# prip-lab/MSU-LatentAFIS

Measured on AMD Instinct MI355X. Metric: latent queries/sec vs 100k rolled gallery, higher is better.
Workload: dtype f32

## Files before the change

include/afis_matcher_taps.h:

```cpp
#ifndef AFIS_MATCHER_TAPS_H
#define AFIS_MATCHER_TAPS_H

#include "afis_matcher.h"

#ifdef __cplusplus
extern "C" {
#endif

int afis_debug_lut(afis_ctx* ctx, const afis_template_view* query, float* out, int32_t* n_rows);
int afis_debug_texture_rowmax(afis_ctx* ctx, const afis_template_view* query, int64_t g,
                              float* val, int32_t* arg, int32_t* n_rows);

int afis_debug_stage_list(afis_ctx* ctx, const afis_template_view* query, int64_t g, int which, int stage,
                          float* sim, int32_t* li, int32_t* ri, int32_t* n);

int afis_debug_atan2_grid(afis_ctx* ctx, int R, float* out);

int afis_debug_graph_arith(afis_ctx* ctx, unsigned long long* out8);
int afis_debug_refine_stats(afis_ctx* ctx, unsigned long long* out8, int reset);

int afis_debug_compact_stats(afis_ctx* ctx, long long* out2);

int afis_debug_rank_subjects(afis_ctx* ctx, afis_subjects* subjects, const float* scores , int n_q, int k,
                             int64_t* subject_id, float* subject_score, int64_t* best_idx);

int afis_debug_rank_hits(afis_ctx* ctx, afis_subjects* subjects, const float* scores , int n_q, float min_score, int cap,
                         int64_t* n_hits , int64_t* out_a , float* out_score , int64_t* out_b );

int afis_debug_rank_latent_hits(afis_ctx* ctx, const float* scores , int n_q, float min_score, int cap, int64_t latent_base,
                                int64_t* n_hits , int64_t* latent_idx , float* score );
int afis_debug_rank_rows(afis_ctx* ctx, afis_subset* subset, const float* scores , int n_q, int k,
                         int64_t* topk_idx , float* topk_score );
int afis_debug_transpose_stats(afis_ctx* ctx, long long* out2);

int afis_debug_phase_cycles(afis_ctx* ctx, unsigned long long* out32, int reset);

#ifdef __cplusplus
}
#endif
#endif
```

msu-latentafis_amd/csrc/afis_taps.cpp:

```cpp
#include "afis_ctx.h"
#include "../../include/afis_matcher_taps.h"

using namespace afis;

static int ensure_codes_cf(afis_ctx* ctx, Shard& sh, int variant)
{
    if ((variant != 6 && variant != 7) || sh.codes_cf_built) return AFIS_OK;
    const int64_t G = sh.gal.G;
    std::vector<int32_t> to((size_t)G + 1), cfb((size_t)G + 1);
    HIPCHK(ctx, hipMemcpyAsync(to.data(), sh.gal.tex_off, to.size() * 4, hipMemcpyDeviceToHost, ctx->stream));
    HIPCHK(ctx, hipStreamSynchronize(ctx->stream));
    int64_t nblk = 0;
    for (int64_t t = 0; t < G; ++t) { cfb[(size_t)t] = (int32_t)nblk; const int64_t n = to[(size_t)t + 1] - to[(size_t)t]; nblk += n > 0 ? (n + 63) / 64 + 1 : 0; }
    cfb[(size_t)G] = (int32_t)nblk;
    if (nblk > 0x7fffffff / 64) return fail(ctx, AFIS_EINVAL, "adc_variant 6 / 7: shard too large for the direct kernel's code stream; split the gallery into more shards");
    HIPCHK(ctx, upload(sh.g_tex_cf_blk, cfb, ctx->stream));
    HIPCHK(ctx, sh.g_tex_codes_cf.ensure(std::max<size_t>((size_t)nblk * 64 * 16, 16)));
    sh.gal.tex_cf_blk = sh.g_tex_cf_blk.as<int32_t>();
    sh.gal.tex_codes_cf = sh.g_tex_codes_cf.as<uint4>();
    HIPCHK(ctx, launch_codes_cf(sh.gal, sh.g_tex_codes_cf.p, ctx->stream));
    HIPCHK(ctx, hipStreamSynchronize(ctx->stream));
    sh.codes_cf_built = true;
    return AFIS_OK;
}

static int direct_rowmax(afis_ctx* ctx, const QueryDev& d, const GalleryDev& g, int variant, int chunk, hipEvent_t after_lut)
{
    HIPCHK(ctx, ctx->lut.ensure(std::max<size_t>((size_t)d.n_tiles * kTileFloats * 4, 16)));
    HIPCHK(ctx, launch_lut_build(d, ctx->codewords.as<float>(), ctx->lut.as<float>(), variant, ctx->stream));
    if (after_lut) HIPCHK(ctx, hipEventRecord(after_lut, ctx->stream));
    HIPCHK(ctx, launch_adc_rowmax(d, g, ctx->lut.as<float>(), chunk, variant, ctx->rm_val.as<float>(), ctx->rm_arg.as<int32_t>(), ctx->stream));
    return AFIS_OK;
}

static int direct_adc_stage(afis_ctx* ctx, Shard& sh, const QueryDev& d, int chunk, hipEvent_t after_lut)
{
    const int rcf = ensure_codes_cf(ctx, sh, ctx->adc_variant);
    if (rcf != AFIS_OK) return rcf;
    return direct_rowmax(ctx, d, sh.gal, ctx->adc_variant, chunk, after_lut);
}
__attribute__((constructor)) static void set_direct_adc_stage() { g_direct_adc_stage = direct_adc_stage; }

extern "C" {

int afis_debug_phase_cycles(afis_ctx* ctx, unsigned long long* out32, int reset)
{
    if (!ctx || !out32) return AFIS_EINVAL;
    HIPCHK(ctx, hipSetDevice(ctx->device));
    HIPCHK(ctx, hipStreamSynchronize(ctx->stream));
    HIPCHK(ctx, read_phase_cycles(out32, reset != 0));
    unsigned long long gph[16];
    HIPCHK(ctx, read_graph_phase_cycles(gph, reset != 0));
    for (int i = 0; i < 8; ++i) { out32[5 + i] = gph[i]; out32[21 + i] = gph[8 + i]; }
    return AFIS_OK;
}

int afis_debug_refine_stats(afis_ctx* ctx, unsigned long long* out8, int reset)
{
    if (!ctx || !out8) return fail(ctx, AFIS_EINVAL, "afis_debug_refine_stats: bad argument");
    HIPCHK(ctx, hipSetDevice(ctx->device));
    HIPCHK(ctx, hipStreamSynchronize(ctx->stream));
    for (int i = 0; i < 8; ++i) out8[i] = 0;
    if (!ctx->mf_stats.p) return AFIS_OK;
    HIPCHK(ctx, hipMemcpy(out8, ctx->mf_stats.p, 64, hipMemcpyDeviceToHost));
    if (reset) HIPCHK(ctx, hipMemset(ctx->mf_stats.p, 0, 64));
    return AFIS_OK;
}

int afis_debug_compact_stats(afis_ctx* ctx, long long* out2)
{
    if (!ctx || !out2) return fail(ctx, AFIS_EINVAL, "afis_debug_compact_stats: bad argument");
    out2[0] = ctx->compact_us; out2[1] = ctx->compact_bytes;
    return AFIS_OK;
}

int afis_debug_rank_subjects(afis_ctx* ctx, afis_subjects* subjects, const float* scores, int n_q, int k, int64_t* subject_id, float* subject_score, int64_t* best_idx)
// ... 227 lines not shown
```

msu-latentafis_amd/csrc/graph.hip:

```cpp
#include "afis_device.h"
#include <type_traits>
#include "atan2f_libm.h"
#include "graph_arith.h"
#include "stdsort_order.h"

namespace afis {

#define AFIS_PI 3.1415926
typedef unsigned long long u64;

#ifdef AFIS_PHASE_TIMING
__device__ u64 g_graph_phase[16];
#define GPH_INIT() u64 gph_t0 = __builtin_readcyclecounter()
#define GPH(i) do { if (threadIdx.x == 0) { const u64 t1_ = __builtin_readcyclecounter(); sm.ph[(i)] += t1_ - gph_t0; gph_t0 = t1_; } } while (0)
#define GPH_T0() const u64 gph_k0 = __builtin_readcyclecounter()
#define GPH_K(i) do { if (threadIdx.x == 0) sm.ph[(i)] += __builtin_readcyclecounter() - gph_k0; } while (0)
#define GPH_ZERO() do { if (threadIdx.x < 16) sm.ph[threadIdx.x] = 0; WSYNC(); } while (0)
#define GPH_FLUSH() do { WSYNC(); if (threadIdx.x < 16 && sm.ph[threadIdx.x]) atomicAdd(&g_graph_phase[threadIdx.x], sm.ph[threadIdx.x]); } while (0)
#else
#define GPH_INIT() do {} while (0)
#define GPH(i) do {} while (0)
#define GPH_T0() do {} while (0)
#define GPH_K(i) do {} while (0)
#define GPH_ZERO() do {} while (0)
// ... 301 lines not shown
    }
    dist = fabsf(d1 - d2);
    return ok;
}
template <bool LOOKUP>
__device__ __forceinline__ bool pair_compatible(const Pt& a, const Pt& o, const float* __restrict__ table)
{
    float s1, s2; bool ok = true;
    if (LOOKUP) {
        const int dx1 = abs(a.lx - o.lx), dx2 = abs(a.rx - o.rx), dy1 = abs(a.ly - o.ly), dy2 = abs(a.ry - o.ry);
        ok = !((dx1 >= kDistN) | (dx2 >= kDistN) | (dy1 >= kDistN) | (dy2 >= kDistN));
        s1 = (float)(256 * (dx1 * dx1 + dy1 * dy1)); s2 = (float)(256 * (dx2 * dx2 + dy2 * dy2));
    } else {
        const float dx1 = (float)(a.lx - o.lx), dx2 = (float)(a.rx - o.rx), dy1 = (float)(a.ly - o.ly), dy2 = (float)(a.ry - o.ry);
        const float p = dx1 * dx1, q = dy1 * dy1, r = dx2 * dx2, s = dy2 * dy2;
        s1 = p + q; s2 = r + s;
    }
    const float d1 = __builtin_amdgcn_sqrtf(s1), d2 = __builtin_amdgcn_sqrtf(s2);
    const float dist = fabsf(d1 - d2);
    const float slack = fmaxf(d1, d2) * 4.76837158e-7f;
    if (fabsf(dist - 30.0f) > slack) return ok && dist < 30.0f;
    float exact;
    pair_dist<LOOKUP>(a, o, table, exact);
    return ok && exact < 30.0f;
}
template <bool RANGE_TEST>
__device__ __forceinline__ bool tex_pair_dist(int2 a, int2 o, float& dist)
{
    float n1, n2;
    pair_n(a, o, n1, n2);
    dist = 16.0f * fabsf(sqrt_rn_int(n1) - sqrt_rn_int(n2));
    return RANGE_TEST ? tex_in_range(a, o) : true;
}
template <bool RANGE_TEST>
__device__ __forceinline__ bool tex_pair_compatible(int2 a, int2 o)
{
    float n1, n2;
    pair_n(a, o, n1, n2);
    const bool ok = RANGE_TEST ? tex_in_range(a, o) : true;
    return pair_compatible_n<true>(n1, n2) && ok;
}

__device__ __forceinline__ float minu_pair_dist(int2 a, int2 o)
{
    float n1, n2;
    pair_n(a, o, n1, n2);
    return fabsf(sqrt_rn_int(n1) - sqrt_rn_int(n2));
}
__device__ __forceinline__ bool minu_pair_compatible(int2 a, int2 o)
{
    float n1, n2;
    pair_n(a, o, n1, n2);
    return pair_compatible_n<false>(n1, n2);
}

__device__ __forceinline__ float h_of_x(float x)
{
    const float q0 = x * 0.04f;
    const float r = fmaf(-q0, 25.0f, x);
    const float h = fmaf(r, 0.04f, q0);
    return __builtin_amdgcn_fmed3f(h, 0.0f, 1.0f);
}
__device__ __forceinline__ float h_value(float dist)
{
    const float x = 30.0f - dist;
    const float q0 = x * 0.04f;
    const float r = fmaf(-q0, 25.0f, x);
    const float h = fmaf(r, 0.04f, q0);
    return __builtin_amdgcn_fmed3f(h, 0.0f, 1.0f);
}

template <class SM, bool LOOKUP, int ITERS, int MODE, int REF_TIE>
__device__ int dist_filter(SM& sm, int num, const float* __restrict__ table, const float* __restrict__ ext, SlabBuf slab)
{
    constexpr bool fast = MODE > 0;
    constexpr bool range_test = MODE == 1;
    auto compat_fast = [](int2 a, int2 o) -> bool { if (LOOKUP) return tex_pair_compatible<range_test>(a, o); return minu_pair_compatible(a, o); };
    auto dist_fast = [](int2 a, int2 o) -> float { float d; if (LOOKUP) { tex_pair_dist<range_test>(a, o, d); return d; } return minu_pair_dist(a, o); };
    constexpr int U = SM::U, W = SM::W, NMAX = SM::NMAX;
    [[maybe_unused]] constexpr int PH = LOOKUP ? 8 : 0;
    GPH_INIT();
    const int lane = threadIdx.x;
    for (int i = lane; i < num * W; i += 64) sm.hb[i / W][i % W] = 0u;
    int2 me[U];
#pragma unroll
    for (int u = 0; u < U; ++u) {
        const int t = lane + 64 * u;
        if (t < SM::N4) { sm.b[t] = t < num ? list_sim(sm, ext, t) : 0.0f; sm.y.cc[t] = 0.0f; }
        me[u] = t < num ? sm.xy[t] : make_int2(0, 0);
    }
    WSYNC();
    const int half = num >> 1;
    const bool even = !(num & 1);
    uint32_t* const hb0 = &sm.hb[0][0];
    auto pair = [&](int2 own, int t, int k, int2 other) {
        if (fast ? compat_fast(own, other) : pair_compatible<LOOKUP>(unpack_xy(own), unpack_xy(other), table)) {
            atomicOr(hb0 + (t * W + (k >> 5)), 1u << (k & 31));
            atomicOr(hb0 + (__umul24(k, W) + (t >> 5)), 1u << (t & 31));
        }
    };
    const int tail0 = num & ~63, R = num - tail0;
    const bool grouped = R > 0 && R <= 32;
    const int n_wide = grouped ? tail0 : num;
    uint32_t kb[U];
    const uint32_t num8 = (uint32_t)num * 8u;
#pragma unroll
    for (int u = 0; u < U; ++u) { const int t = lane + 64 * u; kb[u] = t < num ? (uint32_t)t * 8u : 0u; }
#ifndef AFIS_PAIR_UNROLL
#define AFIS_PAIR_UNROLL 1
#endif
    constexpr int DU = fast ? AFIS_PAIR_UNROLL : 1;
    auto pair_loop = [&](auto ua_tag) {
    constexpr int UA = decltype(ua_tag)::value;
    for (int d = 1; d <= half; d += DU) {
        int2 other[DU][UA];
        int kk[DU][UA];
#pragma unroll
        for (int s2 = 0; s2 < DU; ++s2) {
#pragma unroll
            for (int u = 0; u < UA; ++u) {
                const uint32_t a = kb[u] + 8u;
                kb[u] = min(a, a - num8);
                other[s2][u] = *reinterpret_cast<const int2*>(reinterpret_cast<const char*>(sm.xy) + kb[u]);
                kk[s2][u] = (int)(kb[u] >> 3);
            }
        }
        __builtin_amdgcn_sched_barrier(0);
        if (fast) {
            float n1[DU][UA], n2[DU][UA]; bool hit[DU][UA], near[DU][UA]; bool any_near = false;
#pragma unroll
            for (int s2 = 0; s2 < DU; ++s2) {
#pragma unroll
                for (int u = 0; u < UA; ++u) {
                    pair_n(me[u], other[s2][u], n1[s2][u], n2[s2][u]);
                    hit[s2][u] = pair_compatible_t<LOOKUP>(n1[s2][u], n2[s2][u], near[s2][u]);
                    hit[s2][u] = hit[s2][u] | near[s2][u];
                }
            }
            (void)any_near;
#pragma unroll
            for (int s2 = 0; s2 < DU; ++s2) {
                const bool last = d + s2 == half && even;
#pragma unroll
                for (int u = 0; u < UA; ++u) {
                    const int t = lane + 64 * u, k = kk[s2][u];
                    bool ok = hit[s2][u] && t < n_wide && d + s2 <= half && !(last && t >= half);
                    if (LOOKUP && range_test) ok = ok && tex_in_range(me[u], other[s2][u]);
                    if constexpr (LOOKUP) {
                        const int ts = t < num ? t : 0;
                        atomicOr(hb0 + (ts * W + (k >> 5)), ok ? 1u << (k & 31) : 0u);
                        atomicOr(hb0 + (__umul24(k, W) + (ts >> 5)), ok ? 1u << (ts & 31) : 0u);
                    } else if (ok) {
                        atomicOr(hb0 + (t * W + (k >> 5)), 1u << (k & 31));
                        atomicOr(hb0 + (__umul24(k, W) + (t >> 5)), 1u << (t & 31));
                    }
                }
            }
        } else {
            const bool last = d == half && even;
#pragma unroll
            for (int u = 0; u < UA; ++u) {
                const int t = lane + 64 * u;
                if (t < n_wide && !(last && t >= half)) pair(me[u], t, kk[0][u], other[0][u]);
            }
        }
    }
    };
    const int n_blk = (n_wide + 63) >> 6;
    if (n_blk >= U) pair_loop(std::integral_constant<int, U>{});
    else if (U > 1 && n_blk == U - 1) pair_loop(std::integral_constant<int, (U > 1 ? U - 1 : 1)>{});
    else if (n_blk > 0) pair_loop(std::integral_constant<int, U>{});
    if (grouped) {
        const int sh = R <= 8 ? 3 : R <= 16 ? 4 : 5, RG = 1 << sh, dstep = 64 >> sh;
        const int r = lane & (RG - 1), t = tail0 + r;
        const bool row = r < R;
        const int2 own = row ? sm.xy[t] : make_int2(0, 0);
        int d = 1 + (lane >> sh);
        int k = t + d; k = k >= num ? k - num : k;
        for (int d0 = 1; d0 <= half; d0 += dstep) {
            if (row && d <= half && !(d == half && even && t >= half)) pair(own, t, k, sm.xy[k]);
            d += dstep; k += dstep; k = k >= num ? k - num : k;
        }
    }
    WSYNC();
    GPH(PH + 0);
    int myrow[U], trip[U], rlen[U];
    const int Wn = (num + 31) / 32;
    {
        int cnt[U];
#pragma unroll
        for (int u = 0; u < U; ++u) {
            const int t = lane + 64 * u;
            int c = -1;
            if (t < num) {
                c = 0; for (int w = 0; w < Wn; ++w) c += __popc(sm.hb[t][w]);
                sm.y.os.sel[t] = (short)c;
                c = min(c >> 2, 15);
            }
            cnt[u] = c;
        }
        int base = 0;
        for (int bk = 15; bk >= 0; --bk) {
#pragma unroll
            for (int u = 0; u < U; ++u) {
                const bool in = cnt[u] == bk;
                const u64 m = __ballot(in);
                if (in) sm.y.os.order[base + g_lane_prefix(m)] = (short)(lane + 64 * u);
                base += __popcll(m);
            }
        }
        WSYNC();
#pragma unroll
        for (int u = 0; u < U; ++u) {
            const int p = lane + 64 * u;
            myrow[u] = p < num ? (int)sm.y.os.order[p] : -1;
            rlen[u] = myrow[u] >= 0 ? (int)sm.y.os.sel[myrow[u]] : 0;
// ... 685 lines not shown
```

msu-latentafis_amd/csrc/graph_arith.h:

```cpp
#pragma once
#include "afis_device.h"

namespace afis {

typedef short ga_v2s16 __attribute__((ext_vector_type(2)));
typedef unsigned short ga_v2u16 __attribute__((ext_vector_type(2)));

typedef _Float16 ga_v2h __attribute__((ext_vector_type(2)));

__device__ __forceinline__ int pack_h2(int x, int y) { const ga_v2h v = {(_Float16)(float)x, (_Float16)(float)y}; return __builtin_bit_cast(int, v); }
__device__ __forceinline__ void unpack_h2(int w, int& x, int& y) { const ga_v2h v = __builtin_bit_cast(ga_v2h, w); x = (int)(float)v.x; y = (int)(float)v.y; }

__device__ __forceinline__ float diff_n(int a, int o)
{
    const ga_v2h d = __builtin_bit_cast(ga_v2h, a) - __builtin_bit_cast(ga_v2h, o);
    return __builtin_amdgcn_fdot2(d, d, 0.0f, false);
}
__device__ __forceinline__ void pair_n(int2 a, int2 o, float& n1, float& n2)
{
    const ga_v2h dl = __builtin_bit_cast(ga_v2h, a.x) - __builtin_bit_cast(ga_v2h, o.x);
    const ga_v2h dr = __builtin_bit_cast(ga_v2h, a.y) - __builtin_bit_cast(ga_v2h, o.y);
    asm("v_dot2_f32_f16 %0, %2, %2, 0\n\tv_dot2_f32_f16 %1, %3, %3, 0\n\ts_nop 2" : "=&v"(n1), "=v"(n2) : "v"(dl), "v"(dr));
}
__device__ __forceinline__ bool tex_in_range(int2 a, int2 o)
{
    const ga_v2h dl = __builtin_bit_cast(ga_v2h, a.x) - __builtin_bit_cast(ga_v2h, o.x);
    const ga_v2h dr = __builtin_bit_cast(ga_v2h, a.y) - __builtin_bit_cast(ga_v2h, o.y);
    const float m = fmaxf(fmaxf(fabsf((float)dl.x), fabsf((float)dl.y)), fmaxf(fabsf((float)dr.x), fabsf((float)dr.y)));
    return m < 50.0f;
}

__device__ __forceinline__ float sqrt_rn_int(float x)
{
    const float y = __builtin_fminf(__builtin_fmaxf(__builtin_amdgcn_rsqf(x), 0.0f), 1.0f);
// ... 25 lines not shown
    const float p = n1 * n2;
    const float t = uu - p;
    const float band = __builtin_fmaf(fabsf(uu), 3.814697265625e-6f, c * c * 9.5367431640625e-7f);
    near = !(fabsf(t) > band);
    return t < 0.0f;
}
template <bool TEX>
__device__ __forceinline__ bool pair_compatible_exact(float n1, float n2)
{
    const float d = fabsf(sqrt_rn_pos(n1) - sqrt_rn_pos(n2));
    return TEX ? 16.0f * d < 30.0f : d < 30.0f;
}
template <bool TEX>
__device__ __forceinline__ bool pair_compatible_n(float n1, float n2)
{
    constexpr float c = TEX ? 3.515625f : 900.0f;
    const float s = n1 + n2;
    const float u = __builtin_fmaf(s, 0.5f, -0.5f * c);
    const float uu = u * fabsf(u);
    const float p = n1 * n2;
    const float t = uu - p;
    const float band = __builtin_fmaf(fabsf(uu), 3.814697265625e-6f, c * c * 9.5367431640625e-7f);
    bool hit = t < 0.0f;
    const bool near = !(fabsf(t) > band);
    if (__builtin_amdgcn_ballot_w64(near) != 0ull) {
        if (near) {
            const float d = fabsf(sqrt_rn_pos(n1) - sqrt_rn_pos(n2));
            hit = TEX ? 16.0f * d < 30.0f : d < 30.0f;
        }
    }
    return hit;
}

}
```

msu-latentafis_amd/host/matcher.py:

```python
from __future__ import annotations

import ctypes as C
import glob
import os
from typing import List, Optional, Sequence, Tuple

import numpy as np

from .templates import Codebook, FPTemplate, read_latent, read_rolled

_HERE = os.path.dirname(os.path.abspath(__file__))
LIB_PATH = os.path.join(os.path.dirname(_HERE), "csrc", "libafis_hip.so")
TEST_LIB_PATH = os.path.join(os.path.dirname(_HERE), "csrc", "libafis_hip_test.so")


class AfisError(RuntimeError):
    pass


CASE_SUM, CASE_MAX = 0, 1


class MinutiaeView(C.Structure):
    _fields_ = [("n", C.c_int32), ("x", C.POINTER(C.c_int16)), ("y", C.POINTER(C.c_int16)), ("ori", C.POINTER(C.c_float)),
                ("des_len", C.c_int32), ("des", C.POINTER(C.c_float))]


class TextureView(C.Structure):
    _fields_ = [("n", C.c_int32), ("x", C.POINTER(C.c_int16)), ("y", C.POINTER(C.c_int16)), ("ori", C.POINTER(C.c_float)),
                ("des_len", C.c_int32), ("des", C.POINTER(C.c_float)), ("codes", C.POINTER(C.c_uint8))]


class TemplateView(C.Structure):
    _fields_ = [("n_minu", C.c_int32), ("minu", C.POINTER(MinutiaeView)), ("n_tex", C.c_int32), ("tex", C.POINTER(TextureView))]


class Timing(C.Structure):
    _fields_ = [("lut_ms", C.c_float), ("adc_ms", C.c_float), ("tex_tail_ms", C.c_float), ("minu_ms", C.c_float), ("fuse_ms", C.c_float), ("topk_ms", C.c_float),
                ("total_ms", C.c_float), ("adc_launches", C.c_int32), ("adc_lookups", C.c_int64), ("pairs", C.c_int64), ("adc_bound_ms", C.c_float), ("adc_refine_ms", C.c_float),
                ("cands_ms", C.c_float), ("minu_graph_ms", C.c_float), ("launch_groups", C.c_int32), ("overlapped_groups", C.c_int32),
                ("minu_tasks", C.c_int64), ("minu_fallback_tasks", C.c_int64), ("minu_tasks_small", C.c_int64), ("minu_tasks_medium", C.c_int64), ("minu_tasks_large", C.c_int64),
                ("bound_clock_ghz", C.c_float), ("cands_clock_ghz", C.c_float)]


EXPORTS = ["afis_create", "afis_create_from_codebook", "afis_device_info", "afis_destroy", "afis_last_error", "afis_gallery_add", "afis_gallery_add_dat", "afis_gallery_add_dat_batch", "afis_gallery_reserve",
           "afis_gallery_add_packed", "afis_gallery_commit", "afis_gallery_size", "afis_gallery_reopen", "afis_gallery_remove", "afis_gallery_export", "afis_gallery_save", "afis_gallery_load",
           "afis_gallery_file_info", "afis_gallery_file_names", "afis_rank_list", "afis_search", "afis_search_dat", "afis_queries_upload",
           "afis_subset_create", "afis_subset_free", "afis_search_subset", "afis_search_subset_resident",
           "afis_subjects_create", "afis_subjects_free", "afis_rank_subjects", "afis_rank_hits", "afis_rank_subject_hits", "afis_queries_upload_reserved", "afis_rank_latent_hits",
           "afis_rank_case_hits", "afis_rank_case_subject_hits",
           "afis_labels_create", "afis_labels_free", "afis_rank_hits_filtered", "afis_rank_subject_hits_filtered",
           "afis_search_resident", "afis_queries_free", "afis_correspondences", "afis_match_all_templates", "afis_pq_encode", "afis_encode_rolled_dat", "afis_get_timing", "afis_get_timing2", "afis_set_option", "afis_get_option"]
TAP_EXPORTS = ["afis_debug_lut", "afis_debug_texture_rowmax", "afis_debug_stage_list", "afis_debug_phase_cycles", "afis_debug_atan2_grid", "afis_debug_graph_arith", "afis_debug_refine_stats", "afis_debug_compact_stats", "afis_debug_rank_subjects", "afis_debug_rank_hits", "afis_debug_rank_latent_hits",
               "afis_debug_transpose_stats", "afis_debug_rank_rows"]


def load_library(path: str = LIB_PATH) -> C.CDLL:
    if not os.path.exists(path):
        raise AfisError(f"{path} not found: build it with `make -C msu-latentafis_amd/csrc` (hipcc, gfx950). There is no CPU fallback.")
    lib = C.CDLL(path)
    vp, i32p, i64p, fp = C.c_void_p, C.POINTER(C.c_int32), C.POINTER(C.c_int64), C.POINTER(C.c_float)
    lib.afis_create.argtypes = [C.POINTER(vp), fp, C.c_int, C.c_int, C.c_int, C.c_int]
    lib.afis_create_from_codebook.argtypes = [C.POINTER(vp), C.c_char_p, C.c_size_t, C.c_int]
    lib.afis_destroy.argtypes = [vp]; lib.afis_destroy.restype = None
    lib.afis_last_error.argtypes = [vp]; lib.afis_last_error.restype = C.c_char_p
    lib.afis_rank_list.argtypes = [C.POINTER(C.c_float), C.c_int64, C.c_int, C.c_int, C.POINTER(C.c_int64), C.POINTER(C.c_float)]
    lib.afis_gallery_add.argtypes = [vp, C.POINTER(TemplateView), C.c_int]
    lib.afis_gallery_add_dat.argtypes = [vp, C.c_char_p, C.c_size_t, i32p]
    lib.afis_gallery_reserve.argtypes = [vp, C.c_int64]
    if hasattr(lib, "afis_gallery_add_dat_batch"):
        lib.afis_gallery_add_dat_batch.argtypes = [vp, C.POINTER(C.c_char_p), C.POINTER(C.c_size_t), C.c_int64, i32p]
    lib.afis_gallery_add_packed.argtypes = [vp, C.c_int64, i64p, C.POINTER(C.c_int16), C.POINTER(C.c_int16), fp, fp,
                                            i64p, C.POINTER(C.c_int16), C.POINTER(C.c_int16), fp, C.POINTER(C.c_uint8)]
    lib.afis_gallery_commit.argtypes = [vp, C.c_int64]
    lib.afis_gallery_save.argtypes = [vp, C.c_char_p, C.POINTER(C.c_char_p)]
    lib.afis_gallery_load.argtypes = [vp, C.c_char_p, C.c_int64, C.c_int64]
    lib.afis_gallery_file_info.argtypes = [C.c_char_p, i64p, i64p, i64p, i32p]
    lib.afis_gallery_file_names.argtypes = [C.c_char_p, C.c_int64, C.c_int64, C.c_char_p, C.c_size_t, C.POINTER(C.c_size_t)]
    lib.afis_gallery_size.argtypes = [vp]; lib.afis_gallery_size.restype = C.c_int64
    if hasattr(lib, "afis_gallery_reopen"):
        lib.afis_gallery_reopen.argtypes = [vp]
        lib.afis_gallery_remove.argtypes = [vp, i64p, C.c_int64]
        lib.afis_gallery_export.argtypes = [vp, C.c_char_p, C.POINTER(C.c_char_p)]
    lib.afis_search.argtypes = [vp, C.POINTER(TemplateView), C.c_int, fp, fp, i32p, C.c_int, i64p, fp]
    lib.afis_search_dat.argtypes = [vp, C.POINTER(C.c_char_p), C.POINTER(C.c_size_t), C.c_int, fp, fp, i32p, C.c_int, i64p, fp]
    lib.afis_queries_upload.argtypes = [vp, C.POINTER(TemplateView), C.c_int, C.POINTER(vp)]
    lib.afis_search_resident.argtypes = [vp, vp, fp, fp, i32p, C.c_int, i64p, fp]
# ... 12 lines not shown
    if hasattr(lib, "afis_rank_latent_hits"):
        lib.afis_queries_upload_reserved.argtypes = [vp, C.POINTER(TemplateView), C.c_int, C.c_int64, C.POINTER(vp)]
        lib.afis_rank_latent_hits.argtypes = [vp, C.c_int64, C.c_float, C.c_int, C.c_int64, i64p, i64p, fp]
    if hasattr(lib, "afis_rank_case_hits"):
        lib.afis_rank_case_hits.argtypes = [vp, i64p, C.c_int, C.c_int, C.c_int64, C.c_float, C.c_int, i64p, i64p, i64p, fp]
        lib.afis_rank_case_subject_hits.argtypes = [vp, vp, i64p, C.c_int, C.c_int, C.c_int64, C.c_float, C.c_int, i64p, i64p, i64p, fp]
    if hasattr(lib, "afis_rank_hits_filtered"):
        u64p = C.POINTER(C.c_uint64)
        lib.afis_labels_create.argtypes = [vp, u64p, C.c_int64, C.POINTER(vp)]
        lib.afis_labels_free.argtypes = [vp, vp]; lib.afis_labels_free.restype = None
        lib.afis_rank_hits_filtered.argtypes = [vp, vp, u64p, i64p, i64p, C.c_int, C.c_float, C.c_int, i64p, i64p, fp]
        lib.afis_rank_subject_hits_filtered.argtypes = [vp, vp, vp, u64p, i64p, i64p, C.c_int, C.c_float, C.c_int, i64p, i64p, fp, i64p]
    lib.afis_correspondences.argtypes = [vp, vp, i64p, C.c_int, i32p, C.POINTER(C.c_int16)]
    lib.afis_queries_free.argtypes = [vp, vp]; lib.afis_queries_free.restype = None
    lib.afis_match_all_templates.argtypes = [vp, vp, fp, i32p, i32p]
    lib.afis_pq_encode.argtypes = [vp, fp, C.c_int64, C.POINTER(C.c_uint8)]
    lib.afis_encode_rolled_dat.argtypes = [vp, C.c_char_p, C.c_size_t, C.c_void_p, C.c_size_t, C.POINTER(C.c_size_t), i32p]
    lib.afis_get_timing.argtypes = [vp, C.POINTER(Timing)]
    if hasattr(lib, "afis_get_timing2"):
        lib.afis_get_timing2.argtypes = [vp, C.POINTER(Timing), C.c_size_t]
    lib.afis_set_option.argtypes = [vp, C.c_char_p, C.c_int64]
    if hasattr(lib, "afis_device_info"):
        lib.afis_device_info.argtypes = [C.c_int, C.c_char_p, C.c_size_t, C.c_char_p, C.c_size_t, C.c_char_p, C.c_size_t, i32p]
    if hasattr(lib, "afis_get_option"):
        lib.afis_get_option.argtypes = [vp, C.c_char_p, i64p]
    if hasattr(lib, "afis_debug_stage_list"):
        lib.afis_debug_stage_list.argtypes = [vp, vp, C.c_int64, C.c_int, C.c_int, fp, i32p, i32p, i32p]
        lib.afis_debug_lut.argtypes = [vp, C.POINTER(TemplateView), fp, i32p]
        lib.afis_debug_texture_rowmax.argtypes = [vp, C.POINTER(TemplateView), C.c_int64, fp, i32p, i32p]
        lib.afis_debug_phase_cycles.argtypes = [vp, C.POINTER(C.c_uint64), C.c_int]
        lib.afis_debug_atan2_grid.argtypes = [vp, C.c_int, fp]
    if hasattr(lib, "afis_debug_graph_arith"):
        lib.afis_debug_graph_arith.argtypes = [vp, C.POINTER(C.c_ulonglong)]
    if hasattr(lib, "afis_debug_compact_stats"):
        lib.afis_debug_compact_stats.argtypes = [vp, C.POINTER(C.c_longlong)]
    if hasattr(lib, "afis_debug_refine_stats"):
        lib.afis_debug_refine_stats.argtypes = [vp, C.POINTER(C.c_ulonglong), C.c_int]
    if hasattr(lib, "afis_debug_rank_subjects"):
        lib.afis_debug_rank_subjects.argtypes = [vp, vp, fp, C.c_int, C.c_int, i64p, fp, i64p]
    if hasattr(lib, "afis_debug_rank_hits"):
        lib.afis_debug_rank_hits.argtypes = [vp, vp, fp, C.c_int, C.c_float, C.c_int, i64p, i64p, fp, i64p]
    if hasattr(lib, "afis_debug_rank_latent_hits"):
        lib.afis_debug_rank_latent_hits.argtypes = [vp, fp, C.c_int, C.c_float, C.c_int, C.c_int64, i64p, i64p, fp]
        lib.afis_debug_transpose_stats.argtypes = [vp, C.POINTER(C.c_longlong)]
    if hasattr(lib, "afis_debug_rank_rows"):
        lib.afis_debug_rank_rows.argtypes = [vp, vp, fp, C.c_int, C.c_int, i64p, fp]
    return lib


def _ptr(a: np.ndarray, t):
    return a.ctypes.data_as(C.POINTER(t))


class _Views:

    def __init__(self, templates: Sequence[FPTemplate]):
        self.keep = []
        self.arr = (TemplateView * max(1, len(templates)))()
        for i, t in enumerate(templates):
            mv = (MinutiaeView * max(1, len(t.minu)))()
            for j, m in enumerate(t.minu):
                x = np.ascontiguousarray(m.x, np.int16); y = np.ascontiguousarray(m.y, np.int16)
                o = np.ascontiguousarray(m.ori, np.float32); d = np.ascontiguousarray(m.des, np.float32)
                self.keep += [x, y, o, d]
                mv[j] = MinutiaeView(len(x), _ptr(x, C.c_int16), _ptr(y, C.c_int16), _ptr(o, C.c_float), d.shape[1] if d.ndim == 2 else 0, _ptr(d, C.c_float))
            tv = (TextureView * max(1, len(t.tex)))()
# ... 389 lines not shown
        self._chk(self.lib.afis_encode_rolled_dat(self.ctx, buf, len(buf), out, need.value, C.byref(need), C.byref(rc)))
        return rc.value, out.raw[:need.value]

    def free_queries(self, handle):
        self.lib.afis_queries_free(self.ctx, handle[0])

    def timing(self) -> dict:
        t = Timing()
        if hasattr(self.lib, "afis_get_timing2"):
            self._chk(self.lib.afis_get_timing2(self.ctx, C.byref(t), C.sizeof(Timing)))
        else:
            self._chk(self.lib.afis_get_timing(self.ctx, C.byref(t)))
        return {n: getattr(t, n) for n, _ in Timing._fields_ if n != "reserved_"}

    def _tap(self, name: str):
        if not hasattr(self.lib, name):
            raise AfisError(f"{name} is a parity tap: construct Matcher(..., taps=True) (libafis_hip_test.so); the product library does not export it")
        return getattr(self.lib, name)

    def phase_cycles(self, reset: bool = True):
        out = (C.c_uint64 * 32)()
        self._chk(self._tap("afis_debug_phase_cycles")(self.ctx, out, 1 if reset else 0))
        return list(out)

    def debug_atan2_grid(self, R: int) -> np.ndarray:
        out = np.empty((2 * R + 1, 2 * R + 1), np.float32)
        self._chk(self._tap("afis_debug_atan2_grid")(self.ctx, R, _ptr(out, C.c_float)))
        return out

    def debug_graph_arith(self) -> list:
        out = (C.c_ulonglong * 8)()
        self._chk(self._tap("afis_debug_graph_arith")(self.ctx, out))
        return list(out)

    def refine_stats(self, reset: bool = True) -> dict:
        out = (C.c_ulonglong * 8)()
        self._chk(self._tap("afis_debug_refine_stats")(self.ctx, out, 1 if reset else 0))
        return dict(zip(("pairs", "rows", "rows_evaluated", "cells_evaluated", "rows_evaluated_in_full", "bound_violations"), list(out)[:6]))

    def compact_stats(self):
        out = (C.c_longlong * 2)()
        self._chk(self._tap("afis_debug_compact_stats")(self.ctx, out))
        return int(out[0]), int(out[1])

    def debug_stage_list(self, latent: FPTemplate, g: int, which: int, stage: int):
        v = _Views([latent])
        sim = np.zeros(200, np.float32); li = np.zeros(200, np.int32); ri = np.zeros(200, np.int32); n = C.c_int32(0)
        self._chk(self._tap("afis_debug_stage_list")(self.ctx, v.arr, g, which, stage, _ptr(sim, C.c_float), _ptr(li, C.c_int32), _ptr(ri, C.c_int32), C.byref(n)))
        if n.value < 0:
            return None
        return sim[:n.value], li[:n.value], ri[:n.value]

    def debug_lut(self, latent: FPTemplate) -> np.ndarray:
        v = _Views([latent])
        n = latent.tex[0].n if latent.tex else 0
        out = np.empty((max(n, 1), 16, 256), np.float32); nr = C.c_int32(0)
        self._chk(self._tap("afis_debug_lut")(self.ctx, v.arr, _ptr(out, C.c_float), C.byref(nr)))
        return out[:nr.value]

    def debug_texture_rowmax(self, latent: FPTemplate, g: int):
        v = _Views([latent])
        val = np.zeros(1000, np.float32); arg = np.zeros(1000, np.int32); nr = C.c_int32(0)
        self._chk(self._tap("afis_debug_texture_rowmax")(self.ctx, v.arr, g, _ptr(val, C.c_float), _ptr(arg, C.c_int32), C.byref(nr)))
        return val[:nr.value], arg[:nr.value]

    def load_gallery_dir(self, rolled_path: str) -> List[str]:
# ... 68 lines not shown
```

Baseline: 53.27.

## Compute pair-compatibility bitmaps with MFMA 32x32 tiles instead of pairwise atomics

In fast, non-range-test mode, the graph kernel now builds the pair-compatibility bit matrix with 32x32 tiles. Squared distances come from MFMA f32 outer products, and the hit masks are converted to row words via ballot and v_writelane. This replaces the per-pair loop that issued LDS atomicOr for both symmetric bits. The old loop is moved into a shared helper and is still used for the other modes. A debug tap is added to compare both constructions, since the band test on the MFMA result must agree exactly with the scalar compatibility test.

```diff
diff --git a/include/afis_matcher_taps.h b/include/afis_matcher_taps.h
--- a/include/afis_matcher_taps.h
+++ b/include/afis_matcher_taps.h
@@ -17,6 +17,7 @@
 int afis_debug_atan2_grid(afis_ctx* ctx, int R, float* out);
 
 int afis_debug_graph_arith(afis_ctx* ctx, unsigned long long* out8);
+int afis_debug_pattern(afis_ctx* ctx, int kind, const int16_t* pts , int num, uint32_t* rows_pairs, uint32_t* rows_tiles);
 int afis_debug_refine_stats(afis_ctx* ctx, unsigned long long* out8, int reset);
 
 int afis_debug_compact_stats(afis_ctx* ctx, long long* out2);
diff --git a/msu-latentafis_amd/csrc/afis_taps.cpp b/msu-latentafis_amd/csrc/afis_taps.cpp
--- a/msu-latentafis_amd/csrc/afis_taps.cpp
+++ b/msu-latentafis_amd/csrc/afis_taps.cpp
@@ -1,4 +1,5 @@
 #include "afis_ctx.h"
+#include "graph_arith.h"
 #include "../../include/afis_matcher_taps.h"
 
 using namespace afis;
@@ -41,7 +42,64 @@
 }
 __attribute__((constructor)) static void set_direct_adc_stage() { g_direct_adc_stage = direct_adc_stage; }
 
+template <int NMAX_>
+struct PatternSmem {
+    static constexpr int NMAX = NMAX_, W = (NMAX_ + 31) / 32, U = (NMAX_ + 63) / 64;
+    int2 xy[NMAX_];
+    uint32_t hb[NMAX_][W];
+};
+template <int NMAX, bool TEX>
+__global__ __launch_bounds__(64) void k_debug_pattern(const short4* __restrict__ pts, int num, uint32_t* __restrict__ out)
+{
+    typedef PatternSmem<NMAX> SM;
+    __shared__ SM sm;
+    const int lane = threadIdx.x;
+    uint32_t* const hb0 = &sm.hb[0][0];
+    for (int build = 0; build < 2; ++build) {
+        for (int i = lane; i < NMAX * SM::W; i += 64) hb0[i] = 0u;
+        int2 me[SM::U];
+#pragma unroll
+        for (int u = 0; u < SM::U; ++u) {
+            const int t = lane + 64 * u;
+            me[u] = make_int2(0, 0);
+            if (t < num) { const short4 p = pts[t]; me[u] = make_int2(pack_h2(p.x, p.y), pack_h2(p.z, p.w)); sm.xy[t] = me[u]; }
+        }
+        __syncthreads();
+        if (build == 0) pattern_pair_loop<SM, TEX, TEX ? 2 : 1>(sm, num, me, [](int2, int2) -> bool { return false; });
+        else pattern_tiles<SM, TEX>(sm, num);
+        __syncthreads();
+        for (int i = lane; i < NMAX * SM::W; i += 64) out[build * NMAX * SM::W + i] = hb0[i];
+        __syncthreads();
+    }
+}
+
 extern "C" {
+
+int afis_debug_pattern(afis_ctx* ctx, int kind, const int16_t* pts, int num, uint32_t* rows_pairs, uint32_t* rows_tiles)
+{
+    if (!ctx || !pts || !rows_pairs || !rows_tiles || (kind != 0 && kind != 1)) return fail(ctx, AFIS_EINVAL, "afis_debug_pattern: bad argument");
+    const int nmax = kind ? kTopTex : kTopMinu, hi = kind ? 49 : 2047;
+    if (num < 1 || num > nmax) return fail(ctx, AFIS_EINVAL, "afis_debug_pattern: list length outside [1, 120] (minutiae) / [1, 200] (texture)");
+    for (int i = 0; i < 4 * num; ++i)
+        if (pts[i] < 0 || pts[i] > hi) return fail(ctx, AFIS_EINVAL, "afis_debug_pattern: coordinate outside [0, 2047] (minutiae) / [0, 49] (texture): not a list of the packed paths");
+    HIPCHK(ctx, hipSetDevice(ctx->device));
+    const size_t words = (size_t)nmax * ((nmax + 31) / 32);
+    DevBuf in, out;
+    HIPCHK(ctx, in.ensure((size_t)num * 8));
+    hipError_t e = out.ensure(2 * words * 4);
+    if (e == hipSuccess) e = hipMemcpyAsync(in.p, pts, (size_t)num * 8, hipMemcpyHostToDevice, ctx->stream);
+    if (e == hipSuccess) {
+        if (kind) hipLaunchKernelGGL((k_debug_pattern<kTopTex, true>), dim3(1), dim3(64), 0, ctx->stream, in.as<short4>(), num, out.as<uint32_t>());
+        else hipLaunchKernelGGL((k_debug_pattern<kTopMinu, false>), dim3(1), dim3(64), 0, ctx->stream, in.as<short4>(), num, out.as<uint32_t>());
+        e = hipGetLastError();
+    }
+    if (e == hipSuccess) e = hipMemcpyAsync(rows_pairs, out.p, words * 4, hipMemcpyDeviceToHost, ctx->stream);
+    if (e == hipSuccess) e = hipMemcpyAsync(rows_tiles, out.as<uint32_t>() + words, words * 4, hipMemcpyDeviceToHost, ctx->stream);
+    if (e == hipSuccess) e = hipStreamSynchronize(ctx->stream);
+    in.release(); out.release();
+    if (e != hipSuccess) return fail(ctx, AFIS_EDEVICE, std::string("afis_debug_pattern: ") + hipGetErrorString(e));
+    return AFIS_OK;
+}
 
 int afis_debug_phase_cycles(afis_ctx* ctx, unsigned long long* out32, int reset)
 {
diff --git a/msu-latentafis_amd/csrc/graph.hip b/msu-latentafis_amd/csrc/graph.hip
--- a/msu-latentafis_amd/csrc/graph.hip
+++ b/msu-latentafis_amd/csrc/graph.hip
@@ -357,26 +357,12 @@
     dist = 16.0f * fabsf(sqrt_rn_int(n1) - sqrt_rn_int(n2));
     return RANGE_TEST ? tex_in_range(a, o) : true;
 }
-template <bool RANGE_TEST>
-__device__ __forceinline__ bool tex_pair_compatible(int2 a, int2 o)
-{
-    float n1, n2;
-    pair_n(a, o, n1, n2);
-    const bool ok = RANGE_TEST ? tex_in_range(a, o) : true;
-    return pair_compatible_n<true>(n1, n2) && ok;
-}
 
 __device__ __forceinline__ float minu_pair_dist(int2 a, int2 o)
 {
     float n1, n2;
     pair_n(a, o, n1, n2);
     return fabsf(sqrt_rn_int(n1) - sqrt_rn_int(n2));
-}
-__device__ __forceinline__ bool minu_pair_compatible(int2 a, int2 o)
-{
-    float n1, n2;
-    pair_n(a, o, n1, n2);
-    return pair_compatible_n<false>(n1, n2);
 }
 
 __device__ __forceinline__ float h_of_x(float x)
@@ -400,7 +386,6 @@
 {
     constexpr bool fast = MODE > 0;
     constexpr bool range_test = MODE == 1;
-    auto compat_fast = [](int2 a, int2 o) -> bool { if (LOOKUP) return tex_pair_compatible<range_test>(a, o); return minu_pair_compatible(a, o); };
     auto dist_fast = [](int2 a, int2 o) -> float { float d; if (LOOKUP) { tex_pair_dist<range_test>(a, o, d); return d; } return minu_pair_dist(a, o); };
     constexpr int U = SM::U, W = SM::W, NMAX = SM::NMAX;
     [[maybe_unused]] constexpr int PH = LOOKUP ? 8 : 0;
@@ -415,98 +400,8 @@
         me[u] = t < num ? sm.xy[t] : make_int2(0, 0);
     }
     WSYNC();
-    const int half = num >> 1;
-    const bool even = !(num & 1);
-    uint32_t* const hb0 = &sm.hb[0][0];
-    auto pair = [&](int2 own, int t, int k, int2 other) {
-        if (fast ? compat_fast(own, other) : pair_compatible<LOOKUP>(unpack_xy(own), unpack_xy(other), table)) {
-            atomicOr(hb0 + (t * W + (k >> 5)), 1u << (k & 31));
-            atomicOr(hb0 + (__umul24(k, W) + (t >> 5)), 1u << (t & 31));
-        }
-    };
-    const int tail0 = num & ~63, R = num - tail0;
-    const bool grouped = R > 0 && R <= 32;
-    const int n_wide = grouped ? tail0 : num;
-    uint32_t kb[U];
-    const uint32_t num8 = (uint32_t)num * 8u;
-#pragma unroll
-    for (int u = 0; u < U; ++u) { const int t = lane + 64 * u; kb[u] = t < num ? (uint32_t)t * 8u : 0u; }
-#ifndef AFIS_PAIR_UNROLL
-#define AFIS_PAIR_UNROLL 1
-#endif
-    constexpr int DU = fast ? AFIS_PAIR_UNROLL : 1;
-    auto pair_loop = [&](auto ua_tag) {
-    constexpr int UA = decltype(ua_tag)::value;
-    for (int d = 1; d <= half; d += DU) {
-        int2 other[DU][UA];
-        int kk[DU][UA];
-#pragma unroll
-        for (int s2 = 0; s2 < DU; ++s2) {
-#pragma unroll
-            for (int u = 0; u < UA; ++u) {
-                const uint32_t a = kb[u] + 8u;
-                kb[u] = min(a, a - num8);
-                other[s2][u] = *reinterpret_cast<const int2*>(reinterpret_cast<const char*>(sm.xy) + kb[u]);
-                kk[s2][u] = (int)(kb[u] >> 3);
-            }
-        }
-        __builtin_amdgcn_sched_barrier(0);
-        if (fast) {
-            float n1[DU][UA], n2[DU][UA]; bool hit[DU][UA], near[DU][UA]; bool any_near = false;
-#pragma unroll
-            for (int s2 = 0; s2 < DU; ++s2) {
-#pragma unroll
-                for (int u = 0; u < UA; ++u) {
-                    pair_n(me[u], other[s2][u], n1[s2][u], n2[s2][u]);
-                    hit[s2][u] = pair_compatible_t<LOOKUP>(n1[s2][u], n2[s2][u], near[s2][u]);
-                    hit[s2][u] = hit[s2][u] | near[s2][u];
-                }
-            }
-            (void)any_near;
-#pragma unroll
-            for (int s2 = 0; s2 < DU; ++s2) {
-                const bool last = d + s2 == half && even;
-#pragma unroll
-                for (int u = 0; u < UA; ++u) {
-                    const int t = lane + 64 * u, k = kk[s2][u];
-                    bool ok = hit[s2][u] && t < n_wide && d + s2 <= half && !(last && t >= half);
-                    if (LOOKUP && range_test) ok = ok && tex_in_range(me[u], other[s2][u]);
-                    if constexpr (LOOKUP) {
-                        const int ts = t < num ? t : 0;
-                        atomicOr(hb0 + (ts * W + (k >> 5)), ok ? 1u << (k & 31) : 0u);
-                        atomicOr(hb0 + (__umul24(k, W) + (ts >> 5)), ok ? 1u << (ts & 31) : 0u);
-                    } else if (ok) {
-                        atomicOr(hb0 + (t * W + (k >> 5)), 1u << (k & 31));
-                        atomicOr(hb0 + (__umul24(k, W) + (t >> 5)), 1u << (t & 31));
-                    }
-                }
-            }
-        } else {
-            const bool last = d == half && even;
-#pragma unroll
-            for (int u = 0; u < UA; ++u) {
-                const int t = lane + 64 * u;
-                if (t < n_wide && !(last && t >= half)) pair(me[u], t, kk[0][u], other[0][u]);
-            }
-        }
-    }
-    };
-    const int n_blk = (n_wide + 63) >> 6;
-    if (n_blk >= U) pair_loop(std::integral_constant<int, U>{});
-    else if (U > 1 && n_blk == U - 1) pair_loop(std::integral_constant<int, (U > 1 ? U - 1 : 1)>{});
-    else if (n_blk > 0) pair_loop(std::integral_constant<int, U>{});
-    if (grouped) {
-        const int sh = R <= 8 ? 3 : R <= 16 ? 4 : 5, RG = 1 << sh, dstep = 64 >> sh;
-        const int r = lane & (RG - 1), t = tail0 + r;
-        const bool row = r < R;
-        const int2 own = row ? sm.xy[t] : make_int2(0, 0);
-        int d = 1 + (lane >> sh);
-        int k = t + d; k = k >= num ? k - num : k;
-        for (int d0 = 1; d0 <= half; d0 += dstep) {
-            if (row && d <= half && !(d == half && even && t >= half)) pair(own, t, k, sm.xy[k]);
-            d += dstep; k += dstep; k = k >= num ? k - num : k;
-        }
-    }
+    if constexpr (fast && !range_test) pattern_tiles<SM, LOOKUP>(sm, num);
+    else pattern_pair_loop<SM, LOOKUP, MODE>(sm, num, me, [&](int2 own, int2 other) -> bool { return pair_compatible<LOOKUP>(unpack_xy(own), unpack_xy(other), table); });
     WSYNC();
     GPH(PH + 0);
     int myrow[U], trip[U], rlen[U];
diff --git a/msu-latentafis_amd/csrc/graph_arith.h b/msu-latentafis_amd/csrc/graph_arith.h
--- a/msu-latentafis_amd/csrc/graph_arith.h
+++ b/msu-latentafis_amd/csrc/graph_arith.h
@@ -1,5 +1,6 @@
 #pragma once
 #include "afis_device.h"
+#include <type_traits>
 
 namespace afis {
 
@@ -91,4 +92,182 @@
     return hit;
 }
 
-}
+#ifndef AFIS_PAIR_UNROLL
+#define AFIS_PAIR_UNROLL 1
+#endif
+template <class SM, bool LOOKUP, int MODE, class Generic>
+__device__ __forceinline__ void pattern_pair_loop(SM& sm, int num, const int2 (&me)[SM::U], Generic generic)
+{
+    constexpr bool fast = MODE > 0;
+    constexpr bool range_test = MODE == 1;
+    constexpr int U = SM::U, W = SM::W;
+    const int lane = threadIdx.x;
+    const int half = num >> 1;
+    const bool even = !(num & 1);
+    uint32_t* const hb0 = &sm.hb[0][0];
+    auto pair = [&](int2 own, int t, int k, int2 other) {
+        bool hit;
+        if constexpr (fast) {
+            float n1, n2; bool near;
+            pair_n(own, other, n1, n2);
+            hit = pair_compatible_t<LOOKUP>(n1, n2, near) | near;
+            if (LOOKUP && range_test) hit = hit && tex_in_range(own, other);
+        } else hit = generic(own, other);
+        if (hit) {
+            atomicOr(hb0 + (t * W + (k >> 5)), 1u << (k & 31));
+            atomicOr(hb0 + (__umul24(k, W) + (t >> 5)), 1u << (t & 31));
+        }
+    };
+    const int tail0 = num & ~63, R = num - tail0;
+    const bool grouped = R > 0 && R <= 32;
+    const int n_wide = grouped ? tail0 : num;
+    uint32_t kb[U];
+    const uint32_t num8 = (uint32_t)num * 8u;
+#pragma unroll
+    for (int u = 0; u < U; ++u) { const int t = lane + 64 * u; kb[u] = t < num ? (uint32_t)t * 8u : 0u; }
+    constexpr int DU = fast ? AFIS_PAIR_UNROLL : 1;
+    auto pair_loop = [&](auto ua_tag) {
+    constexpr int UA = decltype(ua_tag)::value;
+    for (int d = 1; d <= half; d += DU) {
+        int2 other[DU][UA];
+        int kk[DU][UA];
+#pragma unroll
+        for (int s2 = 0; s2 < DU; ++s2) {
+#pragma unroll
+            for (int u = 0; u < UA; ++u) {
+                const uint32_t a = kb[u] + 8u;
+                kb[u] = min(a, a - num8);
+                other[s2][u] = *reinterpret_cast<const int2*>(reinterpret_cast<const char*>(sm.xy) + kb[u]);
+                kk[s2][u] = (int)(kb[u] >> 3);
+            }
+        }
+        __builtin_amdgcn_sched_barrier(0);
+        if (fast) {
+            float n1[DU][UA], n2[DU][UA]; bool hit[DU][UA], near[DU][UA];
+#pragma unroll
+            for (int s2 = 0; s2 < DU; ++s2) {
+#pragma unroll
+                for (int u = 0; u < UA; ++u) {
+                    pair_n(me[u], other[s2][u], n1[s2][u], n2[s2][u]);
+                    hit[s2][u] = pair_compatible_t<LOOKUP>(n1[s2][u], n2[s2][u], near[s2][u]);
+                    hit[s2][u] = hit[s2][u] | near[s2][u];
+                }
+            }
+#pragma unroll
+            for (int s2 = 0; s2 < DU; ++s2) {
+                const bool last = d + s2 == half && even;
+#pragma unroll
+                for (int u = 0; u < UA; ++u) {
+                    const int t = lane + 64 * u, k = kk[s2][u];
+                    bool ok = hit[s2][u] && t < n_wide && d + s2 <= half && !(last && t >= half);
+                    if (LOOKUP && range_test) ok = ok && tex_in_range(me[u], other[s2][u]);
+                    if constexpr (LOOKUP) {
+                        const int ts = t < num ? t : 0;
+                        atomicOr(hb0 + (ts * W + (k >> 5)), ok ? 1u << (k & 31) : 0u);
+                        atomicOr(hb0 + (__umul24(k, W) + (ts >> 5)), ok ? 1u << (ts & 31) : 0u);
+                    } else if (ok) {
+                        atomicOr(hb0 + (t * W + (k >> 5)), 1u << (k & 31));
+                        atomicOr(hb0 + (__umul24(k, W) + (t >> 5)), 1u << (t & 31));
+                    }
+                }
+            }
+        } else {
+            const bool last = d == half && even;
+#pragma unroll
+            for (int u = 0; u < UA; ++u) {
+                const int t = lane + 64 * u;
+                if (t < n_wide && !(last && t >= half)) pair(me[u], t, kk[0][u], other[0][u]);
+            }
+        }
+    }
+    };
+    const int n_blk = (n_wide + 63) >> 6;
+    if (n_blk >= U) pair_loop(std::integral_constant<int, U>{});
+    else if (U > 1 && n_blk == U - 1) pair_loop(std::integral_constant<int, (U > 1 ? U - 1 : 1)>{});
+    else if (n_blk > 0) pair_loop(std::integral_constant<int, U>{});
+    if (grouped) {
+        const int sh = R <= 8 ? 3 : R <= 16 ? 4 : 5, RG = 1 << sh, dstep = 64 >> sh;
+        const int r = lane & (RG - 1), t = tail0 + r;
+        const bool row = r < R;
+        const int2 own = row ? sm.xy[t] : make_int2(0, 0);
+        int d = 1 + (lane >> sh);
+        int k = t + d; k = k >= num ? k - num : k;
+        for (int d0 = 1; d0 <= half; d0 += dstep) {
+            if (row && d <= half && !(d == half && even && t >= half)) pair(own, t, k, sm.xy[k]);
+            d += dstep; k += dstep; k = k >= num ? k - num : k;
+        }
+    }
+}
+
+typedef float ga_v16f __attribute__((ext_vector_type(16)));
+template <int V, int N, class F> __device__ __forceinline__ void ga_unroll(F&& f) { f(std::integral_constant<int, V>{}); if constexpr (V + 1 < N) ga_unroll<V + 1, N>(f); }
+template <int L>
+__device__ __forceinline__ void ga_rows_to_lanes(uint32_t& w, unsigned long long m0, unsigned long long m1, unsigned long long m2, unsigned long long m3)
+{
+    asm("s_nop 1\n\t"
+        "v_writelane_b32 %0, %1, %9\n\tv_writelane_b32 %0, %2, %10\n\tv_writelane_b32 %0, %3, %11\n\tv_writelane_b32 %0, %4, %12\n\t"
+        "v_writelane_b32 %0, %5, %13\n\tv_writelane_b32 %0, %6, %14\n\tv_writelane_b32 %0, %7, %15\n\tv_writelane_b32 %0, %8, %16"
+        : "+v"(w)
+        : "s"((uint32_t)m0), "s"((uint32_t)m1), "s"((uint32_t)m2), "s"((uint32_t)m3),
+          "s"((uint32_t)(m0 >> 32)), "s"((uint32_t)(m1 >> 32)), "s"((uint32_t)(m2 >> 32)), "s"((uint32_t)(m3 >> 32)),
+          "n"(L), "n"(L + 1), "n"(L + 2), "n"(L + 3), "n"(L + 4), "n"(L + 5), "n"(L + 6), "n"(L + 7));
+}
+template <class SM, bool TEX>
+__device__ __forceinline__ void pattern_tiles(SM& sm, int num)
+{
+    constexpr float c = TEX ? 3.515625f : 900.0f;
+    const int lane = threadIdx.x, col = lane & 31;
+    const bool hi = lane >= 32;
+    const int nb = (num + 31) >> 5;
+    auto operands = [&](int blk, float& l01, float& lpp, float& r01, float& rpp) {
+        const int t = 32 * blk + col;
+        const int2 p = t < num ? sm.xy[t] : make_int2(0, 0);
+        const ga_v2h l = __builtin_bit_cast(ga_v2h, p.x), r = __builtin_bit_cast(ga_v2h, p.y);
+        const float lx = (float)l.x, ly = (float)l.y, rx = (float)r.x, ry = (float)r.y;
+        lpp = __builtin_fmaf(lx, lx, ly * ly); rpp = __builtin_fmaf(rx, rx, ry * ry);
+        l01 = hi ? ly : lx; r01 = hi ? ry : rx;
+    };
+    for (int I = 0; I < nb; ++I) {
+        float al0, alp, ar0, arp;
+        operands(I, al0, alp, ar0, arp);
+        const float al1 = hi ? 1.0f : alp, ar1 = hi ? 1.0f : arp;
+        const int rows_left = num - 32 * I;
+        for (int J = I; J < nb; ++J) {
+            float bl0, blp, br0, brp;
+            operands(J, bl0, blp, br0, brp);
+            const float bl1 = hi ? blp : 1.0f, br1 = hi ? brp : 1.0f;
+            const ga_v16f z = {0.0f, 0.0f, 0.0f, 0.0f, 0.0f, 0.0f, 0.0f, 0.0f, 0.0f, 0.0f, 0.0f, 0.0f, 0.0f, 0.0f, 0.0f, 0.0f};
+            ga_v16f n1 = __builtin_amdgcn_mfma_f32_32x32x2f32(al0, -2.0f * bl0, z, 0, 0, 0);
+            ga_v16f n2 = __builtin_amdgcn_mfma_f32_32x32x2f32(ar0, -2.0f * br0, z, 0, 0, 0);
+            n1 = __builtin_amdgcn_mfma_f32_32x32x2f32(al1, bl1, n1, 0, 0, 0);
+            n2 = __builtin_amdgcn_mfma_f32_32x32x2f32(ar1, br1, n2, 0, 0, 0);
+            uint32_t w = 0u, tw = 0u;
+            unsigned long long m[16];
+            ga_unroll<0, 16>([&](auto vt) {
+                constexpr int v = decltype(vt)::value;
+                constexpr int r = 8 * (v >> 2) + (v & 3);
+                const float s = n1[v] + n2[v];
+                const float u = __builtin_fmaf(s, 0.5f, -0.5f * c);
+                const float uu = u * fabsf(u);
+                const float p = n1[v] * n2[v];
+                const float t = uu - p;
+                const float band = __builtin_fmaf(fabsf(uu), 3.814697265625e-6f, c * c * 9.5367431640625e-7f);
+                const bool hit = !(t > band);
+                m[v] = __builtin_amdgcn_ballot_w64(hit);
+                tw |= hit ? 1u << r : 0u;
+            });
+            ga_unroll<0, 4>([&](auto at) { constexpr int a = decltype(at)::value; ga_rows_to_lanes<8 * a>(w, m[4 * a], m[4 * a + 1], m[4 * a + 2], m[4 * a + 3]); });
+            const int cols_left = num - 32 * J;
+            uint32_t cm = cols_left >= 32 ? ~0u : (1u << cols_left) - 1u;
+            if (I == J) cm &= ~(1u << col);
+            if (lane < 32 && lane < rows_left) sm.hb[32 * I + lane][J] = w & cm;
+            if (I != J) {
+                tw <<= hi ? 4 : 0;
+                tw |= (uint32_t)__shfl_xor((int)tw, 32);
+                if (lane < 32 && lane < cols_left) sm.hb[32 * J + lane][I] = tw;
+            }
+        }
+    }
+}
+
+}
diff --git a/msu-latentafis_amd/host/matcher.py b/msu-latentafis_amd/host/matcher.py
--- a/msu-latentafis_amd/host/matcher.py
+++ b/msu-latentafis_amd/host/matcher.py
@@ -52,7 +52,7 @@
            "afis_labels_create", "afis_labels_free", "afis_rank_hits_filtered", "afis_rank_subject_hits_filtered",
            "afis_search_resident", "afis_queries_free", "afis_correspondences", "afis_match_all_templates", "afis_pq_encode", "afis_encode_rolled_dat", "afis_get_timing", "afis_get_timing2", "afis_set_option", "afis_get_option"]
 TAP_EXPORTS = ["afis_debug_lut", "afis_debug_texture_rowmax", "afis_debug_stage_list", "afis_debug_phase_cycles", "afis_debug_atan2_grid", "afis_debug_graph_arith", "afis_debug_refine_stats", "afis_debug_compact_stats", "afis_debug_rank_subjects", "afis_debug_rank_hits", "afis_debug_rank_latent_hits",
-               "afis_debug_transpose_stats", "afis_debug_rank_rows"]
+               "afis_debug_transpose_stats", "afis_debug_rank_rows", "afis_debug_pattern"]
 
 
 def load_library(path: str = LIB_PATH) -> C.CDLL:
@@ -131,6 +131,8 @@
         lib.afis_debug_atan2_grid.argtypes = [vp, C.c_int, fp]
     if hasattr(lib, "afis_debug_graph_arith"):
         lib.afis_debug_graph_arith.argtypes = [vp, C.POINTER(C.c_ulonglong)]
+    if hasattr(lib, "afis_debug_pattern"):
+        lib.afis_debug_pattern.argtypes = [vp, C.c_int, C.POINTER(C.c_int16), C.c_int, C.POINTER(C.c_uint32), C.POINTER(C.c_uint32)]
     if hasattr(lib, "afis_debug_compact_stats"):
         lib.afis_debug_compact_stats.argtypes = [vp, C.POINTER(C.c_longlong)]
     if hasattr(lib, "afis_debug_refine_stats"):
@@ -586,6 +588,13 @@
         out = (C.c_ulonglong * 8)()
         self._chk(self._tap("afis_debug_graph_arith")(self.ctx, out))
         return list(out)
+
+    def debug_pattern(self, kind: int, pts: np.ndarray):
+        pts = np.ascontiguousarray(pts, np.int16).reshape(-1, 4)
+        shape = (200, 7) if kind else (120, 4)
+        a = np.zeros(shape, np.uint32); b = np.zeros(shape, np.uint32)
+        self._chk(self._tap("afis_debug_pattern")(self.ctx, kind, _ptr(pts, C.c_int16), len(pts), _ptr(a, C.c_uint32), _ptr(b, C.c_uint32)))
+        return a, b
 
     def refine_stats(self, reset: bool = True) -> dict:
         out = (C.c_ulonglong * 8)()
```

New measurement: 53.69, median of 6. About the same (+0.8%).
